# OnurBasci/TransformerBasedNavierStokeSolver

Hardware: AMD Instinct MI355X
Metric: ns64_train_samples_per_s (higher is better)
Workload: dtype f32

## Files before the change

### transformerbasednavierstokesolver_amd/csrc/pa2d_gemm.hip

```cpp
#include "pa2d_gemm_common.h"
#include <string.h>


static Pa2dEnv read_env() {
    auto is = [](const char* n, const char* pre) { const char* e = getenv(n); return e && strncmp(e, pre, strlen(pre)) == 0; };
    auto num = [](const char* n, int dflt) { const char* e = getenv(n); return (e && e[0]) ? atoi(e) : dflt; };
    Pa2dEnv v;
    v.conv_halo = is("PA2D_CONV_HALO", "o") ? 0 : (is("PA2D_CONV_HALO", "f") ? 2 : 1);
    v.mc_big_off = is("PA2D_MC_BIG", "o") ? 1 : 0;
    v.kc_bk16 = num("PA2D_KC_BK", 0) == 16 ? 1 : 0;
    v.mc_bk = num("PA2D_MC_BK", 16) == 32 ? 32 : 16;
    v.mc_splits = num("PA2D_MC_SPLITS", 0);
    v.mcb_splits = num("PA2D_MCB_SPLITS", 0);
    v.lin_dw_split = is("PA2D_LIN_DW_SPLIT", "of") ? 0 : 1;
    v.lin_panel = is("PA2D_LIN_PANEL", "of") ? 0 : 1;
    v.lin_rowpanel = is("PA2D_LIN_ROWPANEL", "of") ? 0 : 1;
    v.lin_small_split = is("PA2D_LIN_SMALL_SPLIT", "of") ? 0 : 1;
    v.conv_mfma16 = num("PA2D_CONV_MFMA", 16) == 32 ? 0 : 1;
    v.conv_ahead = num("PA2D_CONV_AHEAD", 1) == 0 ? 0 : 1;
    v.mc_mfma16 = num("PA2D_MC_MFMA", 16) == 32 ? 0 : 1;
    v.split_big = num("PA2D_SPLIT_BIG", 1);
    v.slice_map = is("PA2D_SLICE_MAP", "l") ? 0 : 1;
    v.default_engine = is("PA2D_GEMM", "f") ? 0 : (is("PA2D_GEMM", "b") ? 2 : 1);
    v.tail_panel = num("PA2D_TAIL_PANEL", 0);
    return v;
}
static Pa2dEnv g_env = read_env();
const Pa2dEnv& pa2d_env() { return g_env; }


static int kc_bk(bool im2col, int Cin) {
    if (im2col && pa2d_env().kc_bk16) return 16;
    return (!im2col || (Cin % 32) == 0) ? 32 : 16;
}
static KCTile kc_tile(int M, int N, bool im2col, int Cin) {
    const int tiles_m = ceil_div(M, 128);
    const long long t128 = (long long)tiles_m * ceil_div(N, 128);
    const long long t12864 = (long long)tiles_m * ceil_div(N, 64);
    const int bk = kc_bk(im2col, Cin);
    if (N > 64 && t128 >= 384) return {128, 128, bk};
    if (t12864 >= 384 || M <= 64) return {128, 64, bk};
    return {64, 64, bk};
}
static bool use_split(int engine, int N, bool im2col, int Cin) {
    const int m = engine;
    if (m == 1) return im2col && N > 64 && (Cin % 32) == 0;
    if (m == 2) return N > 64 && (!im2col || (Cin % 32) == 0);
    return false;
}
static bool kc_split_small_applies(const KCParams& p, bool im2col) {
    if (!pa2d_env().lin_small_split || im2col || p.io_bf16 || p.engine != 1) return false;
    if ((p.K % 32) != 0 || p.K < 64 || p.N < 64 || p.M < 256) return false;
    return (long long)ceil_div(p.M, 128) * ceil_div(p.N, 128) < 384;
}
static int persistent_mode(const KCParams& p) {
    const bool gelu = p.act == ACT_GELU, has_res = p.res != nullptr;
    if (p.epi == 0) return 0;
    if (gelu && !has_res && (p.epi == (EPI_ACT | EPI_STORE_PRE) || p.epi == EPI_ACT)) return 1;
    if (gelu && !has_res && p.epi == EPI_MUL_DACT && !p.bias) return 2;
    return -1;
}
static bool panel_applies(const KCParams& p, bool im2col) {
    if (!pa2d_env().lin_panel || im2col) return false;
    if (p.io_bf16 || (p.engine != 1 && p.engine != 2)) return false;
    if ((p.K % 32) != 0 || p.N < 64) return false;
    if (persistent_mode(p) < 0) return false;
    if (p.epi == EPI_ACT && p.aux) return false;
    return (long long)(p.M / 256) * ceil_div(p.N, 128) >= 256;
}
static size_t rowpanel_image_bytes(int N, int K, int engine) {
    if (engine != 1 || (K != 128 && K != 256) || N < 128 || N > 1024 || (N % 128) != 0) return 0;
    return (size_t)N * K * 6;
}
static bool rowpanel_applies(const KCParams& p) {
    if (!pa2d_env().lin_rowpanel || p.io_bf16) return false;
    if (rowpanel_image_bytes(p.N, p.K, p.engine) == 0) return false;
    if (persistent_mode(p) < 0 || (p.epi == EPI_ACT && p.aux)) return false;
    if ((p.lda & 3) || (p.ldc & 3) || (p.res && (p.ldres & 3)) || (p.aux && (p.ldaux & 3))) return false;
    return p.M / 128 >= 256;
}
static bool conv_halo_applies(const KCParams& p) {
    const int pol = pa2d_env().conv_halo;
    if (p.taps == 27) return false;
    if (pol == 0 || !p.apre || (p.Cin % 32) != 0 || p.H <= 0 || p.W <= 0 || (p.M % (p.H * p.W)) != 0) return false;
    const long long tiles = (long long)(p.M / (p.H * p.W)) * ceil_div(p.H, KC_HALO_TH) * ceil_div(p.W, KC_HALO_TW) * ceil_div(p.N, 128);
    return pol == 2 || tiles >= 512;
}

KCChoice plan_kc(const KCParams& p, bool im2col) {
    KCChoice c = {};
    c.mode = c.tail_family = c.tail_bm = c.tail_bn = -1;
    c.out_bf16 = p.io_bf16;
    c.reads_b = true;
    c.wimg_bytes = im2col ? 0 : rowpanel_image_bytes(p.N, p.K, p.engine);
    const int nt = p.engine == 2 ? 1 : 3;
    if (!im2col && p.wimg && rowpanel_applies(p)) {
        c.family = KC_ROWPANEL; c.bm = 128; c.bn = 64; c.bk = 64; c.nt = 3;
    } else if (panel_applies(p, im2col)) {
        c.family = KC_PANEL; c.bm = 256; c.bn = 128; c.bk = 32; c.nt = nt;
    } else if (p.io_bf16 || use_split(p.engine, p.N, im2col, p.Cin)) {
        c.family = KC_SPLIT; c.bm = 128; c.bn = 128; c.bk = 32; c.nt = nt;
        c.a_planes = im2col ? p.apre != 0 : p.io_bf16 != 0;
        if (im2col) c.pack = KC_PACK_PLANES;
        if (im2col ? !p.apre : p.engine != 2) c.rc = PA2D_ERR_ARG;
        else if (p.io_bf16 && (p.taps == 27 || p.engine != 2 || (!im2col && (p.K % 32) != 0))) c.rc = PA2D_ERR_UNSUPPORTED;
        else if (im2col && conv_halo_applies(p)) {
            c.family = KC_HALO; c.bm = 256;
            c.mfma16 = nt == 3 && pa2d_env().conv_mfma16 && (p.N % 4) == 0 && (p.ldc % 4) == 0;
            c.ahead = c.mfma16 && pa2d_env().conv_ahead;
        } else if (im2col && !p.io_bf16 && nt == 3) {
            const int tiles_n = ceil_div(p.N, 128);
            if (pa2d_env().split_big && (p.M % 256) == 0 && (long long)(p.M / 256) * tiles_n >= 512) c.bm = 256;
            else if ((long long)ceil_div(p.M, 128) * tiles_n < 256) c.bm = 64;
        }
    } else if (kc_split_small_applies(p, im2col)) {
        c.family = KC_SPLIT_SMALL; c.bm = 64; c.bn = 64; c.bk = 32; c.nt = 3;
    } else {
        const KCTile t = kc_tile(p.M, p.N, im2col, p.Cin);
        c.family = KC_EXACT; c.bm = t.bm; c.bn = t.bn; c.bk = t.bk;
        if (im2col) c.pack = t.bk == 32 ? KC_PACK_F32_32 : KC_PACK_F32_16;
    }
    if (c.family == KC_PANEL || c.family == KC_ROWPANEL) {
        c.mode = persistent_mode(p);
        c.head_rows = p.M - p.M % c.bm;
        if (c.head_rows < p.M) {
            KCParams pt = p;
            pt.wimg = nullptr;
            pt.M = p.M - c.head_rows;
            const KCChoice t = plan_kc(pt, false);
            c.tail_family = t.family; c.tail_bm = t.bm; c.tail_bn = t.bn;
        }
        c.reads_b = c.family == KC_PANEL || c.head_rows < p.M;
    }
    return c;
}

static bool kc_extents(KCParams& p, bool im2col, const KCChoice& c) {
    const unsigned long long lim = 0xFFFFFFF0ull;
    const unsigned long long es = p.io_bf16 ? 2ull : 4ull;
    unsigned long long ab = ((unsigned long long)(p.M - 1) * p.lda + (im2col ? p.Cin : p.K)) * 4ull;
    unsigned long long bb = ((unsigned long long)(p.N - 1) * p.ldb + p.K) * 4ull;
    const unsigned long long cb = ((unsigned long long)(p.M - 1) * p.ldc + p.N) * es;
    const unsigned long long rb = p.res ? ((unsigned long long)(p.M - 1) * p.ldres + p.N) * es : 0ull;
    const unsigned long long xb = p.aux ? ((unsigned long long)(p.M - 1) * p.ldaux + p.N) * es : 0ull;
    if (ab >= lim || bb >= lim || cb >= lim || rb >= lim || xb >= lim) return false;
    if (c.a_planes) ab = im2col ? (unsigned long long)p.M * (p.Cin / 32) * c.nt * 64 : ab / 2;
    if (c.pack == KC_PACK_PLANES) bb = (unsigned long long)p.N * (p.K / 32) * c.nt * 64;
    if (ab >= lim) return false;
    p.a_bytes = (unsigned)ab; p.b_bytes = (unsigned)bb;
    p.c_bytes = (unsigned)cb; p.res_bytes = (unsigned)rb; p.aux_bytes = (unsigned)xb;
    return true;
}

static int launch_head_tail(const KCParams& p_in, const KCParams& p, const KCChoice& c, hipStream_t st) {
    int rc;
    if (c.family == KC_ROWPANEL && p.wsrc) {
        rc = launch_pack_weight_image(p.wsrc, p.wsn, p.wsk, p.wimg, p.N, p.K, st);
        if (rc) return rc;
    }
    KCParams ph = p;
    ph.M = c.head_rows;
    rc = c.family == KC_ROWPANEL ? launch_kc_rowpanel(ph, c, st) : launch_kc_panel(ph, c, st);
    if (rc || c.head_rows == p.M) return rc;
    KCParams pt = p_in;
    pt.wimg = nullptr;
    pt.M = p.M - c.head_rows;
    pt.A = p.A + (size_t)c.head_rows * p.lda;
    pt.C = p.C + (size_t)c.head_rows * p.ldc;
    if (p.res) pt.res = p.res + (size_t)c.head_rows * p.ldres;
    if (p.aux) pt.aux = p.aux + (size_t)c.head_rows * p.ldaux;
    return launch_kc(pt, false, st);
}

// ... 258 lines not shown
```

### transformerbasednavierstokesolver_amd/csrc/pa2d_gemm_mc_planes.hip

```cpp
#include "pa2d_gemm_common.h"
#include "pa2d_bf16_split.h"

struct MCPlanesParams {
    const void* PA; int chA;
    const void* PB; int chB;
    float* slab;
    int Mi, Nj, Mk, chunks_per_split, splits, H, W, Cin;
    unsigned a_bytes, b_bytes;
    int taps;
    long long lda, ldb;
    float* colsum;
};

__device__ __forceinline__ unsigned img_off(int row, int ch) {
    return 256u * row + 16u * (ch ^ (((row & 3) << 2) | ((row >> 2) & 3)));
}

#define MC16_FRAG(base_, t_, pl_)                                                                         \
    __builtin_bit_cast(bf16x8, __builtin_shufflevector(                                                   \
        __builtin_amdgcn_ds_read_tr16_b64_v4i16((lds_s16x4*)(smem + ((base_[0] ^ ((unsigned)(t_) << 5)) + (pl_) * PIMG))), \
        __builtin_amdgcn_ds_read_tr16_b64_v4i16((lds_s16x4*)(smem + ((base_[1] ^ ((unsigned)(t_) << 5)) + (pl_) * PIMG))), \
        0, 1, 2, 3, 4, 5, 6, 7))

template <int NT, int KS, bool F32SRC = false, bool MF16 = false>
// ... 108 lines not shown
    _Pragma("unroll") for (int op = 0; op < 2; ++op) MC_SPLIT_ROW8(NT, rg[op * 2], rg[op * 2 + 1], op == 0 && do_cs, cs, pk[op])
#define MP16_WRITE(buf_)                                                                                  \
    _Pragma("unroll") for (int op = 0; op < 2; ++op) _Pragma("unroll") for (int pl = 0; pl < NT; ++pl)    \
        *reinterpret_cast<bf16x8*>(smem + (buf_) * STAGE + flds + (op * NT + pl) * PIMG) = pk[op][pl];
        const int nst = c_end - c_begin, steps = (nst + 1) >> 1;
        if (nst > 0) {
            MP_LOAD(c_begin)
            MP16_CONVERT()
            MP16_WRITE(0)
            MP_LOAD(c_begin + 1)
            MP16_CONVERT()
            MP16_WRITE(1)
            if (steps > 1) { MP_LOAD(c_begin + 2) }
        }
        __syncthreads();
        int sp = 0, sq = 1, sr = 2;
        for (int k = 0; k < steps; ++k) {
            const bool has_next = k + 1 < steps;
            const unsigned lo = (unsigned)((kq >> 1) ? sq : sp) * (unsigned)STAGE;
            const unsigned ua[2] = {fa[0] + lo, fa[1] + lo};
            const unsigned ub[2] = {fb[0] + lo + NT * PIMG, fb[1] + lo + NT * PIMG};
            bf16x8 xf[4][NT];
#pragma unroll
            for (int j = 0; j < 4; ++j)
#pragma unroll
                for (int pl = 0; pl < NT; ++pl) xf[j][pl] = MC16_FRAG(ub, j, pl);
            bf16x8 afc[NT], afn[NT];
#pragma unroll
            for (int pl = 0; pl < NT; ++pl) afc[pl] = MC16_FRAG(ua, 0, pl);
#pragma unroll
            for (int ib = 0; ib < 4; ++ib) {
                if (ib < 3) {
#pragma unroll
                    for (int pl = 0; pl < NT; ++pl) afn[pl] = MC16_FRAG(ua, ib + 1, pl);
                }
                if (ib == 1 && has_next) {
                    MP16_CONVERT()
                    MP16_WRITE(sr)
                    MP_LOAD(c_begin + 2 * k + 3)
                }
                if (ib == 3) {
                    if (has_next) {
                        MP16_CONVERT()
                        if (k + 2 < steps) { MP_LOAD(c_begin + 2 * k + 4) }
                    }
                    __syncthreads();
                    if (has_next) { MP16_WRITE(sp) }
                }
                MP16_MMA(ib, afc)
#pragma unroll
                for (int pl = 0; pl < NT; ++pl) afc[pl] = afn[pl];
            }
            __syncthreads();
            const int t = sp;
            sp = sr;
            sr = sq;
            sq = t;
        }
#undef MP16_CONVERT
#undef MP16_WRITE
#undef MP16_MMA
        if (do_cs) {
            float* sm = reinterpret_cast<float*>(smem);
#pragma unroll
            for (int e = 0; e < 8; ++e) sm[frow * 128 + fc8 * 8 + e] = cs[e];
            mc_colsum_reduce<128, 16>(sm, tid, ti, split, p.Mi, p.colsum);
        }
        float* out = p.slab + (size_t)split * p.Mi * p.Nj;
#pragma unroll
        for (int j = 0; j < 4; ++j) {
            const int col = tj * 128 + wn * 64 + j * 16 + 4 * kq;
#pragma unroll
            for (int ib = 0; ib < 4; ++ib) {
                const int row = ti * 128 + wm * 64 + ib * 16 + (lane & 15);
                if (row < p.Mi && col < p.Nj) *reinterpret_cast<f32x4*>(out + (size_t)row * p.Nj + col) = acc[ib][j];
            }
        }
        return;
    }

    f32x16 acc[2][2];
#pragma unroll
    for (int i = 0; i < 2; ++i)
#pragma unroll
        for (int j = 0; j < 2; ++j)
#pragma unroll
            for (int r = 0; r < 16; ++r) acc[i][j][r] = 0.f;

    const int g = lane >> 4, q4 = (lane & 15) >> 2, pq = lane & 3;
    unsigned fa[2][2], fb[2][2];
#pragma unroll
    for (int t = 0; t < 2; ++t)
#pragma unroll
        for (int r = 0; r < 2; ++r) {
            const int row = 8 * (g >> 1) + 4 * r + q4;
            const int cha = ((wm * 64 + t * 32) >> 3) + 2 * (g & 1) + (pq >> 1);
            const int chb = ((wn * 64 + t * 32) >> 3) + 2 * (g & 1) + (pq >> 1);
            fa[t][r] = img_off(row, cha) + 8u * (pq & 1);
            fb[t][r] = img_off(row, chb) + 8u * (pq & 1);
        }

    if (c_begin < c_end) {
        MP_LOAD(c_begin)
        MP_STORE(0)
    }
    __syncthreads();
    for (int c = c_begin; c < c_end; c += KS) {
        const int buf = ((c - c_begin) / KS) & 1;
        if (c + KS < c_end) { MP_LOAD(c + KS) }
#pragma unroll
        for (int ks = 0; ks < KS; ++ks) {
        const unsigned char* st = smem + buf * STAGE + ks * PIMG;
        bf16x8 af[2][NT], bf[2][NT];
#pragma unroll
        for (int t = 0; t < 2; ++t)
#pragma unroll
            for (int pl = 0; pl < NT; ++pl) {
                af[t][pl] = tr_frag(st + pl * KS * PIMG, fa[t][0], fa[t][1]);
                bf[t][pl] = tr_frag(st + (NT + pl) * KS * PIMG, fb[t][0], fb[t][1]);
            }
#pragma unroll
        for (int i = 0; i < 2; ++i)
#pragma unroll
            for (int j = 0; j < 2; ++j) split_terms(af[i], bf[j], acc[i][j]);
        }
        if (c + KS < c_end) { MP_STORE(buf ^ 1) }
        __syncthreads();
    }
#undef MP_LOAD
#undef MP_STORE

    if constexpr (F32SRC) {
        if (do_cs) {
            float* sm = reinterpret_cast<float*>(smem);
#pragma unroll
            for (int e = 0; e < 8; ++e) sm[frow * 128 + fc8 * 8 + e] = cs[e];
            mc_colsum_reduce<128, 16>(sm, tid, ti, split, p.Mi, p.colsum);
        }
    }
    float* out = p.slab + (size_t)split * p.Mi * p.Nj;
    const int col0 = tj * 128 + wn * 64 + (lane & 31);
    const int row0 = ti * 128 + wm * 64 + 4 * (lane >> 5);
#pragma unroll
    for (int j = 0; j < 2; ++j)
#pragma unroll
        for (int i = 0; i < 2; ++i)
#pragma unroll
            for (int r = 0; r < 16; ++r) {
                const int row = row0 + i * 32 + (r & 3) + 8 * (r >> 2);
                if (!F32SRC || (row < p.Mi && col0 + j * 32 < p.Nj)) out[(size_t)row * p.Nj + col0 + j * 32] = acc[i][j][r];
            }
}

template <int NT, int KS, bool MF16 = false>
__global__ __launch_bounds__(512, 1) void gemm_mc_planes_big_kernel(const MCPlanesParams p, const int per_xcd) {
    constexpr int PIMG = 8192;
    constexpr int STAGE = 2 * NT * KS * PIMG;
    constexpr int NP = (2 * NT * KS * 512) / 512;
    extern __shared__ __attribute__((aligned(16))) unsigned char smem[];

    const int tid = threadIdx.x, lane = tid & 63, wave = tid >> 6;
    const int tiles_i = (p.Mi + 255) / 256, tiles_j = (p.Nj + 255) / 256;
    const int tiles = tiles_i * tiles_j;
    const int lin = (blockIdx.x & 7) * per_xcd + (blockIdx.x >> 3);
    if ((int)(blockIdx.x >> 3) >= per_xcd || lin >= tiles * p.splits) return;
    const int split = lin / tiles, t_ = lin - split * tiles;
    const int ti = t_ / tiles_j, tj = t_ - ti * tiles_j;
    const int wm = wave >> 2, wn = wave & 3;
    const int total_chunks = (p.Mk + 15) / 16;
    const int c_begin = split * p.chunks_per_split;
    const int c_end = min(total_chunks, c_begin + p.chunks_per_split);
    const int HW = p.taps == 1 ? 1 : p.H * p.W;

    const __amdgpu_buffer_rsrc_t ra_rsrc = __builtin_amdgcn_make_buffer_rsrc(const_cast<void*>(p.PA), 0, p.a_bytes, 0x00020000);
    const __amdgpu_buffer_rsrc_t rb_rsrc = __builtin_amdgcn_make_buffer_rsrc(const_cast<void*>(p.PB), 0, p.b_bytes, 0x00020000);

    const int row16 = tid >> 5, cgrp = (tid & 31) >> 2, piece = tid & 3;
    const bool colok_a = ti * 256 + cgrp * 32 < p.Mi;
    const unsigned goff_a = (unsigned)((((ti * 256) >> 5) + cgrp) * NT * 64 + piece * 16);
    const int jc = tj * 256 + cgrp * 32;
    const int tap = p.taps == 1 ? 4 : jc / p.Cin;
    const bool colok_b = jc < p.Nj;
    const unsigned goff_b = (unsigned)((p.taps == 1 ? (jc >> 5) : ((jc - tap * p.Cin) >> 5)) * NT * 64 + piece * 16);
    const int tap_dy = tap / 3 - 1, tap_dx = tap - (tap / 3) * 3 - 1, tap_shift = tap_dy * p.W + tap_dx;
    const unsigned pitch_a = (unsigned)(p.chA * NT * 64), pitch_b = (unsigned)(p.chB * NT * 64);
    const unsigned lds_off = 512u * row16 + 16u * ((unsigned)(cgrp * 4 + piece) ^ (unsigned)(((row16 & 3) << 2) | ((row16 >> 2) & 3)));
#define MB_LOAD(c_, RG)                                                                                   \
    {                                                                                                     \
        _Pragma("unroll") for (int ks = 0; ks < KS; ++ks) {                                               \
            const int m_ = ((c_) + ks) * 16 + row16;                                                      \
            const bool okr_ = m_ < p.Mk && (c_) + ks < c_end;             \
            bool okb_ = okr_ && colok_b;                                                                  \
            int mm_ = m_;                                                                                 \
            if (p.taps != 1) {       \
                okb_ = okb_ && (unsigned)(ly + tap_dy) < (unsigned)p.H && (unsigned)(lx + tap_dx) < (unsigned)p.W; \
                mm_ = m_ + tap_shift;                                                                     \
                lx += 16;                                                                                 \
                while (lx >= p.W) { lx -= p.W; ++ly; }                                                    \
                while (ly >= p.H) ly -= p.H;                                                              \
            }                                                                                             \
            const unsigned oa_ = (okr_ && colok_a) ? (unsigned)m_ * pitch_a + goff_a : OOB_OFF;           \
            const unsigned ob_ = okb_ ? (unsigned)mm_ * pitch_b + goff_b : OOB_OFF;                       \
            _Pragma("unroll") for (int pl = 0; pl < NT; ++pl) {                                           \
                RG[pl * KS + ks] = __builtin_amdgcn_raw_buffer_load_b128(ra_rsrc, oa_ == OOB_OFF ? OOB_OFF : oa_ + pl * 64u, 0, 0); \
                RG[(NT + pl) * KS + ks] = __builtin_amdgcn_raw_buffer_load_b128(rb_rsrc, ob_ == OOB_OFF ? OOB_OFF : ob_ + pl * 64u, 0, 0); \
            }                                                                                             \
        }                                                                                                 \
    }
#define MB_STORE(buf_, RG)                                                                                \
    {                                                                                                     \
        _Pragma("unroll") for (int s = 0; s < NP; ++s)                                                    \
            *reinterpret_cast<u32x4*>(smem + (buf_) * STAGE + s * PIMG + lds_off) = RG[s];                \
    }
    u32x4 rg0[NP];
    int ly = 0, lx = 0;
    if (p.taps != 1) {
        const int n0 = (c_begin * 16 + row16) % HW;
        ly = n0 / p.W;
        lx = n0 - ly * p.W;
    }

    if constexpr (MF16) {
        static_assert(NT == 3 && KS == 1, "the 16x16x32 form is written for the split engine");
        f32x4 acc[8][4];
#pragma unroll
        for (int i = 0; i < 8; ++i)
#pragma unroll
            for (int j = 0; j < 4; ++j) acc[i][j] = f32x4{0.f, 0.f, 0.f, 0.f};
        const int kq = lane >> 4, q4 = (lane & 15) >> 2, pq = lane & 3;
        unsigned fa[2], fb[2];
#pragma unroll
        for (int r = 0; r < 2; ++r) {
            const int row = 8 * (kq & 1) + 4 * r + q4;
            const unsigned swz = (unsigned)(((row & 3) << 2) | ((row >> 2) & 3));
            fa[r] = 512u * row + 16u * ((unsigned)(wm * 16 + (pq >> 1)) ^ swz) + 8u * (pq & 1);
            fb[r] = 512u * row + 16u * ((unsigned)(wn * 8 + (pq >> 1)) ^ swz) + 8u * (pq & 1);
        }
#define MB16_MMA(ib_, AF) _Pragma("unroll") for (int j = 0; j < 4; ++j) split_terms(AF, xf[j], acc[ib_][j]);
        const int nst = c_end - c_begin, steps = (nst + 1) >> 1;
        if (nst > 0) {
            MB_LOAD(c_begin, rg0)
            MB_STORE(0, rg0)
            MB_LOAD(c_begin + 1, rg0)
            MB_STORE(1, rg0)
            if (steps > 1) MB_LOAD(c_begin + 2, rg0)
        }
        __syncthreads();
        int sp = 0, sq = 1, sr = 2;
        for (int k = 0; k < steps; ++k) {
            const unsigned lo = (unsigned)((kq >> 1) ? sq : sp) * (unsigned)STAGE;
            const unsigned ua[2] = {fa[0] + lo, fa[1] + lo};
            const unsigned ub[2] = {fb[0] + lo + NT * PIMG, fb[1] + lo + NT * PIMG};
            bf16x8 xf[4][NT];
#pragma unroll
            for (int j = 0; j < 4; ++j)
#pragma unroll
                for (int pl = 0; pl < NT; ++pl) xf[j][pl] = MC16_FRAG(ub, j, pl);
            bf16x8 afc[NT], afn[NT];
#pragma unroll
            for (int pl = 0; pl < NT; ++pl) afc[pl] = MC16_FRAG(ua, 0, pl);
#pragma unroll
            for (int ib = 0; ib < 8; ++ib) {
                if (ib < 7) {
#pragma unroll
                    for (int pl = 0; pl < NT; ++pl) afn[pl] = MC16_FRAG(ua, ib + 1, pl);
                }
                if (ib == 4) {
                    MB_STORE(sr, rg0)
                    MB_LOAD(c_begin + 2 * k + 3, rg0)
                }
                if (ib == 7) {
                    __syncthreads();
                    MB_STORE(sp, rg0)
                    MB_LOAD(c_begin + 2 * k + 4, rg0)
                }
                MB16_MMA(ib, afc)
#pragma unroll
                for (int pl = 0; pl < NT; ++pl) afc[pl] = afn[pl];
            }
            __syncthreads();
            const int t = sp;
            sp = sr;
            sr = sq;
            sq = t;
        }
#undef MB16_MMA
        float* out = p.slab + (size_t)split * p.Mi * p.Nj;
#pragma unroll
        for (int j = 0; j < 4; ++j) {
            const int col = tj * 256 + wn * 64 + j * 16 + 4 * kq;
            if (col >= p.Nj) continue;
#pragma unroll
            for (int ib = 0; ib < 8; ++ib) {
                const int row = ti * 256 + wm * 128 + ib * 16 + (lane & 15);
                if (row < p.Mi) *reinterpret_cast<f32x4*>(out + (size_t)row * p.Nj + col) = acc[ib][j];
            }
        }
        return;
    }

    f32x16 acc[4][2];
#pragma unroll
    for (int i = 0; i < 4; ++i)
#pragma unroll
        for (int j = 0; j < 2; ++j)
#pragma unroll
            for (int r = 0; r < 16; ++r) acc[i][j][r] = 0.f;

    const int g = lane >> 4, q4 = (lane & 15) >> 2, pq = lane & 3;
    unsigned fa[4][2], fb[2][2];
#pragma unroll
    for (int r = 0; r < 2; ++r) {
        const int row = 8 * (g >> 1) + 4 * r + q4;
        const unsigned swz = (unsigned)(((row & 3) << 2) | ((row >> 2) & 3));
#pragma unroll
        for (int t = 0; t < 4; ++t) {
            const int cha = ((wm * 128 + t * 32) >> 3) + 2 * (g & 1) + (pq >> 1);
            fa[t][r] = 512u * row + 16u * ((unsigned)cha ^ swz) + 8u * (pq & 1);
        }
#pragma unroll
        for (int t = 0; t < 2; ++t) {
            const int chb = ((wn * 64 + t * 32) >> 3) + 2 * (g & 1) + (pq >> 1);
            fb[t][r] = 512u * row + 16u * ((unsigned)chb ^ swz) + 8u * (pq & 1);
        }
    }

#define MB_COMPUTE(buf_)                                                                                  \
    _Pragma("unroll") for (int ks = 0; ks < KS; ++ks) {                                                   \
        const unsigned char* st = smem + (buf_) * STAGE + ks * PIMG;                                      \
        bf16x8 af[4][NT], bf[2][NT];                                                                      \
        _Pragma("unroll") for (int pl = 0; pl < NT; ++pl) {                                               \
            _Pragma("unroll") for (int t = 0; t < 4; ++t)                                                 \
                af[t][pl] = tr_frag(st + pl * KS * PIMG, fa[t][0], fa[t][1]);                             \
            _Pragma("unroll") for (int t = 0; t < 2; ++t)                                                 \
                bf[t][pl] = tr_frag(st + (NT + pl) * KS * PIMG, fb[t][0], fb[t][1]);                      \
        }                                                                                                 \
        _Pragma("unroll") for (int i = 0; i < 4; ++i)                                                     \
            _Pragma("unroll") for (int j = 0; j < 2; ++j) split_terms(af[i], bf[j], acc[i][j]);           \
    }
    if (c_begin < c_end) {
        MB_LOAD(c_begin, rg0)
        MB_STORE(0, rg0)
        if (c_begin + KS < c_end) MB_LOAD(c_begin + KS, rg0)
    }
    __syncthreads();
    for (int c = c_begin; c < c_end; c += KS) {
        const int buf = ((c - c_begin) / KS) & 1;
        if (c + KS < c_end) {
            MB_STORE(buf ^ 1, rg0)
            if (c + 2 * KS < c_end) MB_LOAD(c + 2 * KS, rg0)
        }
        MB_COMPUTE(buf)
        __syncthreads();
    }
#undef MB_COMPUTE
#undef MB_LOAD
#undef MB_STORE

    float* out = p.slab + (size_t)split * p.Mi * p.Nj;
    const int col0 = tj * 256 + wn * 64 + (lane & 31);
    const int row0 = ti * 256 + wm * 128 + 4 * (lane >> 5);
    MC_STORE_TILES(4, 2)
}

template <typename K>
static int launch_big(K kernel, int smem, const MCPlanesParams& p, int wgs, hipStream_t st) {
    const int per_xcd = ceil_div(wgs, 8);
    return launch_lds(kernel, dim3(per_xcd * 8), dim3(512), smem, st, p, per_xcd);
}

int launch_wgrad_planes(const MCDesc& d, const MCChoice& c, unsigned a_bytes, unsigned b_bytes, float* slab, hipStream_t st) {
    const int NT = d.engine == 2 ? 1 : 3;
    const bool mf16 = NT == 3 && pa2d_env().mc_mfma16 && (reinterpret_cast<uintptr_t>(slab) & 15) == 0;
    MCPlanesParams p = {};
    p.PA = d.A; p.PB = d.B; p.slab = slab; p.a_bytes = a_bytes; p.b_bytes = b_bytes;
    p.Mi = d.Mi; p.Nj = d.Nj; p.Mk = d.Mk; p.chunks_per_split = c.pl.chunks_per_split; p.splits = c.pl.splits;
    p.H = d.H; p.W = d.W; p.Cin = d.Cin; p.taps = d.taps;
    if (c.kernel == MC_K_PLANES256) {
        p.chA = d.Mi / 32; p.chB = d.Cin / 32;
        const int wgs = ceil_div(p.Mi, 256) * ceil_div(p.Nj, 256) * c.pl.splits;
        int rc;
        if (mf16) rc = launch_big(&gemm_mc_planes_big_kernel<3, 1, true>, 3 * 2 * 3 * 1 * 8192, p, wgs, st);
        else if (NT == 3) rc = launch_big(&gemm_mc_planes_big_kernel<3, 1>, 2 * 2 * 3 * 1 * 8192, p, wgs, st);
        else rc = launch_big(&gemm_mc_planes_big_kernel<1, 4>, 2 * 2 * 1 * 4 * 8192, p, wgs, st);
        return rc;
    }
    if (!c.pl.big) return PA2D_ERR_UNSUPPORTED;
    const dim3 grid(ceil_div(d.Mi, 128) * ceil_div(d.Nj, 128) * c.pl.splits);
    if (c.kernel == MC_K_PLANES128) {
        if ((d.Mi % 128) || (d.Cin % 128) || d.taps != 9) return PA2D_ERR_UNSUPPORTED;
        p.chA = d.Mi / 32; p.chB = d.Cin / 32;
        if (NT == 3) hipLaunchKernelGGL((gemm_mc_planes_kernel<3, 1>), grid, dim3(256), 0, st, p);
        else hipLaunchKernelGGL((gemm_mc_planes_kernel<1, 4>), grid, dim3(256), 0, st, p);
    } else {
        p.lda = d.lda; p.ldb = d.ldb; p.colsum = d.colsum;
        if (mf16 && (d.Nj % 4) == 0) hipLaunchKernelGGL((gemm_mc_planes_kernel<3, 1, true, true>), grid, dim3(256), 0, st, p);
        else if (NT == 3) hipLaunchKernelGGL((gemm_mc_planes_kernel<3, 1, true>), grid, dim3(256), 0, st, p);
        else hipLaunchKernelGGL((gemm_mc_planes_kernel<1, 4, true>), grid, dim3(256), 0, st, p);
    }
    PA2D_CHECK_LAUNCH();
    return PA2D_OK;
}
```

### transformerbasednavierstokesolver_amd/csrc/pa2d_internal.h

```cpp
#pragma once
#include <hip/hip_runtime.h>
#include <stdint.h>

typedef float f32x16 __attribute__((ext_vector_type(16)));
typedef float f32x4 __attribute__((ext_vector_type(4)));

#define PA2D_OK 0
#define PA2D_ERR_ARG 1001
#define PA2D_ERR_UNSUPPORTED 1002
#define PA2D_ERR_WORKSPACE 1003

#define PA2D_CHECK_LAUNCH()                         \
    do {                                            \
        hipError_t e__ = hipGetLastError();         \
        if (e__ != hipSuccess) return (int)e__;     \
    } while (0)

enum { ACT_NONE = 0, ACT_GELU = 1, ACT_TANH = 2, ACT_SIGMOID = 3, ACT_RELU = 4, ACT_SOFTPLUS = 5,
       ACT_ELU = 6, ACT_SILU = 7 };

__device__ __forceinline__ float normal_cdf(float x, float& e_out) {
#pragma clang fp contract(off)
    const float z = fabsf(x) * 0.70710678118654752440f;
    const float t = __builtin_amdgcn_rcpf(fmaf(0.3275911f, z, 1.0f));
    float poly = fmaf(1.061405429f, t, -1.453152027f);
    poly = fmaf(poly, t, 1.421413741f);
    poly = fmaf(poly, t, -0.284496736f);
    poly = fmaf(poly, t, 0.254829592f);
    const float e = __builtin_amdgcn_exp2f(-z * z * 1.44269504088896340736f);
    e_out = e;
    const float hq = 0.5f * poly * t * e;
    return x < 0.f ? hq : 1.0f - hq;
}
__device__ __forceinline__ float gelu_exact(float x) {
#pragma clang fp contract(off)
    float e;
    return x * normal_cdf(x, e);
}
__device__ __forceinline__ float dgelu_exact(float x) {
#pragma clang fp contract(off)
    float e;
    const float cdf = normal_cdf(x, e);
    return fmaf(x * 0.39894228040143267794f, e, cdf);
}

__device__ __forceinline__ float act_fwd(int id, float x) {
    switch (id) {
        case ACT_GELU: return gelu_exact(x);
        case ACT_TANH: return tanhf(x);
        case ACT_SIGMOID: return 1.0f / (1.0f + expf(-x));
        case ACT_RELU: return x > 0.f ? x : 0.f;
        case ACT_SOFTPLUS: return x > 20.f ? x : log1pf(expf(x));
        case ACT_ELU: return x > 0.f ? x : expm1f(x);
        case ACT_SILU: return x / (1.0f + expf(-x));
        default: return x;
    }
}

__device__ __forceinline__ float act_bwd(int id, float x) {
    switch (id) {
        case ACT_GELU: return dgelu_exact(x);
        case ACT_TANH: { const float t = tanhf(x); return 1.0f - t * t; }
        case ACT_SIGMOID: { const float s = 1.0f / (1.0f + expf(-x)); return s * (1.0f - s); }
        case ACT_RELU: return x > 0.f ? 1.f : 0.f;
        case ACT_SOFTPLUS: return x > 20.f ? 1.f : 1.0f / (1.0f + expf(-x));
        case ACT_ELU: return x > 0.f ? 1.f : expf(x);
        case ACT_SILU: { const float s = 1.0f / (1.0f + expf(-x)); return s * (1.0f + x * (1.0f - s)); }
        default: return 1.f;
    }
}

__device__ __forceinline__ float wave_sum(float v) {
#pragma unroll
    for (int o = 32; o > 0; o >>= 1) v += __shfl_xor(v, o, 64);
    return v;
}
__device__ __forceinline__ float wave_max(float v) {
#pragma unroll
    for (int o = 32; o > 0; o >>= 1) v = fmaxf(v, __shfl_xor(v, o, 64));
    return v;
}

typedef unsigned int u32x4 __attribute__((ext_vector_type(4)));
#define OOB_OFF 0xFFFFFFFFu

__device__ __forceinline__ __amdgpu_buffer_rsrc_t make_rsrc(const float* base, unsigned bytes) {
    return __builtin_amdgcn_make_buffer_rsrc(const_cast<float*>(base), 0, bytes, 0x00020000);
}
__device__ __forceinline__ float4 buf_load4(__amdgpu_buffer_rsrc_t r, unsigned voff) {
    const u32x4 v = __builtin_amdgcn_raw_buffer_load_b128(r, voff, 0, 0);
    return make_float4(__uint_as_float(v.x), __uint_as_float(v.y), __uint_as_float(v.z), __uint_as_float(v.w));
}


__device__ __forceinline__ float buf_load1(__amdgpu_buffer_rsrc_t r, unsigned voff) {
    return __uint_as_float(__builtin_amdgcn_raw_buffer_load_b32(r, voff, 0, 0));
}
__device__ __forceinline__ void buf_store1(__amdgpu_buffer_rsrc_t r, unsigned voff, float v) {
    __builtin_amdgcn_raw_buffer_store_b32(__float_as_uint(v), r, voff, 0, 0);
}

__device__ __forceinline__ float2 buf_load2(__amdgpu_buffer_rsrc_t r, unsigned voff) {
    typedef unsigned int u32x2_ __attribute__((ext_vector_type(2)));
    const u32x2_ v = __builtin_amdgcn_raw_buffer_load_b64(r, voff, 0, 0);
    return make_float2(__uint_as_float(v.x), __uint_as_float(v.y));
}
__device__ __forceinline__ void buf_store4(__amdgpu_buffer_rsrc_t r, unsigned voff, float4 v) {
    u32x4 u = {__float_as_uint(v.x), __float_as_uint(v.y), __float_as_uint(v.z), __float_as_uint(v.w)};
    __builtin_amdgcn_raw_buffer_store_b128(u, r, voff, 0, 0);
}

#define PA2D_ACT_SAVE_DERIVATIVE_BIT 0x100

struct Pa2dEnv {
    int conv_halo;
    int mc_big_off;
    int kc_bk16;
    int mc_bk;
    int mc_splits;
    int mcb_splits;
    int lin_dw_split;
    int lin_panel;
    int conv_mfma16;
    int conv_ahead;
    int mc_mfma16;
    int lin_small_split;
    int lin_rowpanel;
    int split_big;
    int slice_map;
    int default_engine;
    int tail_panel;
};
const Pa2dEnv& pa2d_env();

static inline int pa2d_zero(void* p, size_t bytes, hipStream_t st) {
    if (!p || !bytes) return PA2D_OK;
    return (int)hipMemsetAsync(p, 0, bytes, st);
}
static inline int ceil_div(int a, int b) { return (a + b - 1) / b; }
static inline long long ceil_div_ll(long long a, long long b) { return (a + b - 1) / b; }

struct ReduceSegs { int nseg; long long begin[5]; float* dst[4]; };
int pa2d_launch_reduce_segs(const float* slab, int nslab, long long count, const ReduceSegs& segs, int accumulate,
                            hipStream_t st);

typedef __bf16 bf16_t;
template <typename T> struct Act;
template <> struct Act<float> {
    static constexpr unsigned ES = 4;
    static __device__ __forceinline__ float4 ld4(const float* p) { return *reinterpret_cast<const float4*>(p); }
    static __device__ __forceinline__ void st4(float* p, float4 v) { *reinterpret_cast<float4*>(p) = v; }
    static __device__ __forceinline__ float ld1(const float* p) { return *p; }
    static __device__ __forceinline__ float4 bld4(__amdgpu_buffer_rsrc_t r, unsigned off) { return buf_load4(r, off); }
    static __device__ __forceinline__ float2 bld2(__amdgpu_buffer_rsrc_t r, unsigned off) { return buf_load2(r, off); }
    static __device__ __forceinline__ float bld1(__amdgpu_buffer_rsrc_t r, unsigned off) { return buf_load1(r, off); }
    static __device__ __forceinline__ float bld1s(__amdgpu_buffer_rsrc_t r, unsigned off, unsigned soff) {
        return __uint_as_float(__builtin_amdgcn_raw_buffer_load_b32(r, off, soff, 0));
    }
    static __device__ __forceinline__ void bst4(__amdgpu_buffer_rsrc_t r, unsigned off, float4 v) { buf_store4(r, off, v); }
    static __device__ __forceinline__ void bst1(__amdgpu_buffer_rsrc_t r, unsigned off, float v) { buf_store1(r, off, v); }
};
__device__ __forceinline__ float bf16_bits_to_f32(unsigned short b) { return __uint_as_float((unsigned)b << 16); }
__device__ __forceinline__ unsigned short f32_to_bf16_bits(float x) {
    const bf16_t h = (bf16_t)x;
    return __builtin_bit_cast(unsigned short, h);
}
__device__ __forceinline__ unsigned pack_bf16x2(float lo, float hi) {
    return (unsigned)f32_to_bf16_bits(lo) | ((unsigned)f32_to_bf16_bits(hi) << 16);
}
template <> struct Act<bf16_t> {
    static constexpr unsigned ES = 2;
    static __device__ __forceinline__ float4 unpack4(uint2 q) {
        return make_float4(__uint_as_float(q.x << 16), __uint_as_float(q.x & 0xFFFF0000u), __uint_as_float(q.y << 16),
                           __uint_as_float(q.y & 0xFFFF0000u));
    }
    static __device__ __forceinline__ float4 ld4(const bf16_t* p) { return unpack4(*reinterpret_cast<const uint2*>(p)); }
    static __device__ __forceinline__ void st4(bf16_t* p, float4 v) {
        *reinterpret_cast<uint2*>(p) = make_uint2(pack_bf16x2(v.x, v.y), pack_bf16x2(v.z, v.w));
    }
    static __device__ __forceinline__ float ld1(const bf16_t* p) { return (float)*p; }
    static __device__ __forceinline__ float4 bld4(__amdgpu_buffer_rsrc_t r, unsigned off) {
        typedef unsigned int u32x2_ __attribute__((ext_vector_type(2)));
        const u32x2_ q = __builtin_amdgcn_raw_buffer_load_b64(r, off, 0, 0);
        return unpack4(make_uint2(q.x, q.y));
    }
    static __device__ __forceinline__ float2 bld2(__amdgpu_buffer_rsrc_t r, unsigned off) {
        const unsigned q = __builtin_amdgcn_raw_buffer_load_b32(r, off, 0, 0);
        return make_float2(__uint_as_float(q << 16), __uint_as_float(q & 0xFFFF0000u));
    }
    static __device__ __forceinline__ float bld1(__amdgpu_buffer_rsrc_t r, unsigned off) {
        return bf16_bits_to_f32(__builtin_amdgcn_raw_buffer_load_b16(r, off, 0, 0));
    }
    static __device__ __forceinline__ float bld1s(__amdgpu_buffer_rsrc_t r, unsigned off, unsigned soff) {
        return bf16_bits_to_f32(__builtin_amdgcn_raw_buffer_load_b16(r, off, soff, 0));
    }
    static __device__ __forceinline__ void bst4(__amdgpu_buffer_rsrc_t r, unsigned off, float4 v) {
        typedef unsigned int u32x2_ __attribute__((ext_vector_type(2)));
        const u32x2_ q = {pack_bf16x2(v.x, v.y), pack_bf16x2(v.z, v.w)};
        __builtin_amdgcn_raw_buffer_store_b64(q, r, off, 0, 0);
    }
    static __device__ __forceinline__ void bst1(__amdgpu_buffer_rsrc_t r, unsigned off, float v) {
        __builtin_amdgcn_raw_buffer_store_b16(f32_to_bf16_bits(v), r, off, 0, 0);
    }
};
__device__ __forceinline__ __amdgpu_buffer_rsrc_t make_rsrc_v(const void* base, unsigned bytes) {
    return __builtin_amdgcn_make_buffer_rsrc(const_cast<void*>(base), 0, bytes, 0x00020000);
}

__device__ __forceinline__ bool slice_decode(int xcd_map, int B, int heads, int nchunk, int& b, int& hh, int& chunk, int& bid) {
    const int total = B * heads * nchunk;
    int L;
    if (xcd_map) {
        const int per = (total + 7) >> 3;
        if ((int)(blockIdx.x >> 3) >= per) return false;
        L = (int)(blockIdx.x & 7) * per + (int)(blockIdx.x >> 3);
        if (L >= total) return false;
        hh = L % heads;
        chunk = (L / heads) % nchunk;
        b = L / (heads * nchunk);
    } else {
        L = (int)blockIdx.x;
        if (L >= total) return false;
        chunk = L % nchunk;
        hh = (L / nchunk) % heads;
        b = L / (nchunk * heads);
    }
    bid = (b * heads + hh) * nchunk + chunk;
    return true;
}
static inline int slice_grid(int total) { return ((total + 7) / 8) * 8; }
```

Baseline: 71.62.

## Stage big multi-channel GEMM tiles via buffer-load-to-LDS DMA with chained MFMA issue

Adds a DMA staging path for the 256x256 multi-channel planes GEMM kernel. Global tiles are loaded straight into LDS with buffer_load ... lds (inline asm driving m0) rather than through registers and ds_write. The XOR swizzle moves into the per-thread source chunk index, and A fragments are preloaded into a larger register array. An optional chained mode puts scheduling barriers between MFMA groups. Both are on by default via env flags; this frees VGPRs and removes LDS store instructions, at the cost of hand-written asm, a changed sync placement and more register use for A fragments.

```diff
diff --git a/transformerbasednavierstokesolver_amd/csrc/pa2d_gemm.hip b/transformerbasednavierstokesolver_amd/csrc/pa2d_gemm.hip
--- a/transformerbasednavierstokesolver_amd/csrc/pa2d_gemm.hip
+++ b/transformerbasednavierstokesolver_amd/csrc/pa2d_gemm.hip
@@ -19,6 +19,8 @@
     v.conv_mfma16 = num("PA2D_CONV_MFMA", 16) == 32 ? 0 : 1;
     v.conv_ahead = num("PA2D_CONV_AHEAD", 1) == 0 ? 0 : 1;
     v.mc_mfma16 = num("PA2D_MC_MFMA", 16) == 32 ? 0 : 1;
+    v.mc_dma = num("PA2D_MC_DMA", 1) == 0 ? 0 : 1;
+    v.mc_chain = num("PA2D_MC_CHAIN", 1) == 0 ? 0 : 1;
     v.split_big = num("PA2D_SPLIT_BIG", 1);
     v.slice_map = is("PA2D_SLICE_MAP", "l") ? 0 : 1;
     v.default_engine = is("PA2D_GEMM", "f") ? 0 : (is("PA2D_GEMM", "b") ? 2 : 1);
diff --git a/transformerbasednavierstokesolver_amd/csrc/pa2d_gemm_mc_planes.hip b/transformerbasednavierstokesolver_amd/csrc/pa2d_gemm_mc_planes.hip
--- a/transformerbasednavierstokesolver_amd/csrc/pa2d_gemm_mc_planes.hip
+++ b/transformerbasednavierstokesolver_amd/csrc/pa2d_gemm_mc_planes.hip
@@ -284,7 +284,10 @@
             }
 }
 
-template <int NT, int KS, bool MF16 = false>
+#ifndef MB_MID
+#define MB_MID 5
+#endif
+template <int NT, int KS, bool MF16 = false, bool DMA = false, bool CHAIN = false>
 __global__ __launch_bounds__(512, 1) void gemm_mc_planes_big_kernel(const MCPlanesParams p, const int per_xcd) {
     constexpr int PIMG = 8192;
     constexpr int STAGE = 2 * NT * KS * PIMG;
@@ -307,7 +310,11 @@
     const __amdgpu_buffer_rsrc_t ra_rsrc = __builtin_amdgcn_make_buffer_rsrc(const_cast<void*>(p.PA), 0, p.a_bytes, 0x00020000);
     const __amdgpu_buffer_rsrc_t rb_rsrc = __builtin_amdgcn_make_buffer_rsrc(const_cast<void*>(p.PB), 0, p.b_bytes, 0x00020000);
 
-    const int row16 = tid >> 5, cgrp = (tid & 31) >> 2, piece = tid & 3;
+    static_assert(!DMA || MF16, "LDS-DMA staging is written for the 16x16x32 pipeline");
+    static_assert(!CHAIN || DMA, "the chained issue order needs the registers that DMA staging frees");
+    const int row16 = tid >> 5;
+    const int lchunk = DMA ? (tid & 31) ^ (((row16 & 3) << 2) | ((row16 >> 2) & 3)) : (tid & 31);
+    const int cgrp = lchunk >> 2, piece = lchunk & 3;
     const bool colok_a = ti * 256 + cgrp * 32 < p.Mi;
     const unsigned goff_a = (unsigned)((((ti * 256) >> 5) + cgrp) * NT * 64 + piece * 16);
     const int jc = tj * 256 + cgrp * 32;
@@ -344,7 +351,45 @@
         _Pragma("unroll") for (int s = 0; s < NP; ++s)                                                    \
             *reinterpret_cast<u32x4*>(smem + (buf_) * STAGE + s * PIMG + lds_off) = RG[s];                \
     }
-    u32x4 rg0[NP];
+#define MB_DMA(c_, buf_)                                                                                  \
+    {                                                                                                     \
+        const int m_ = (c_) * 16 + row16;                                                                 \
+        const bool okr_ = m_ < p.Mk && (c_) < c_end;                                                      \
+        bool okb_ = okr_ && colok_b;                                                                      \
+        int mm_ = m_;                                                                                     \
+        if (p.taps != 1) {                                                                                \
+            okb_ = okb_ && (unsigned)(ly + tap_dy) < (unsigned)p.H && (unsigned)(lx + tap_dx) < (unsigned)p.W; \
+            mm_ = m_ + tap_shift;                                                                         \
+            lx += 16;                                                                                     \
+            while (lx >= p.W) { lx -= p.W; ++ly; }                                                        \
+            while (ly >= p.H) ly -= p.H;                                                                  \
+        }                                                                                                 \
+        const unsigned oa_ = (okr_ && colok_a) ? (unsigned)m_ * pitch_a + goff_a : OOB_OFF;               \
+        const unsigned ob_ = okb_ ? (unsigned)mm_ * pitch_b + goff_b : OOB_OFF;                           \
+        const unsigned va_[NT] = {oa_, oa_ == OOB_OFF ? OOB_OFF : oa_ + 64u, oa_ == OOB_OFF ? OOB_OFF : oa_ + 128u}; \
+        const unsigned vb_[NT] = {ob_, ob_ == OOB_OFF ? OOB_OFF : ob_ + 64u, ob_ == OOB_OFF ? OOB_OFF : ob_ + 128u}; \
+        unsigned keep_;                                                                                   \
+        asm volatile(MB_DMA_ASM                                                                           \
+                     : "=&s"(keep_)                                                                       \
+                     : "s"(lds_base + (unsigned)(buf_) * (unsigned)STAGE), "s"(dma_ra), "s"(dma_rb),      \
+                       "v"(va_[0]), "v"(va_[1]), "v"(va_[2]), "v"(vb_[0]), "v"(vb_[1]), "v"(vb_[2])       \
+                     : "memory", "scc");                                                                  \
+    }
+#define MB_DMA_ASM                                                                                        \
+    "s_nop 4\n\ts_mov_b32 %0, m0\n\ts_mov_b32 m0, %1\n\ts_nop 0\n\t"                                      \
+    "buffer_load_dwordx4 %4, %2, 0 offen lds\n\ts_add_u32 m0, m0, 0x2000\n\ts_nop 0\n\t"                  \
+    "buffer_load_dwordx4 %5, %2, 0 offen lds\n\ts_add_u32 m0, m0, 0x2000\n\ts_nop 0\n\t"                  \
+    "buffer_load_dwordx4 %6, %2, 0 offen lds\n\ts_add_u32 m0, m0, 0x2000\n\ts_nop 0\n\t"                  \
+    "buffer_load_dwordx4 %7, %3, 0 offen lds\n\ts_add_u32 m0, m0, 0x2000\n\ts_nop 0\n\t"                  \
+    "buffer_load_dwordx4 %8, %3, 0 offen lds\n\ts_add_u32 m0, m0, 0x2000\n\ts_nop 0\n\t"                  \
+    "buffer_load_dwordx4 %9, %3, 0 offen lds\n\ts_mov_b32 m0, %0"
+#define MB_DMA_WAIT() asm volatile("s_waitcnt vmcnt(0)" ::: "memory")
+    static_assert(!DMA || (NT == 3 && PIMG == 0x2000), "MB_DMA_ASM is written out for six 8 KB images");
+    typedef __attribute__((address_space(3))) unsigned char lds_char;
+    const unsigned lds_base = (unsigned)(uintptr_t)(lds_char*)smem + (unsigned)__builtin_amdgcn_readfirstlane(wave) * 1024u;
+    const u32x4 dma_ra = {(unsigned)(uintptr_t)p.PA, (unsigned)((uintptr_t)p.PA >> 32) & 0xFFFFu, p.a_bytes, 0x00020000u};
+    const u32x4 dma_rb = {(unsigned)(uintptr_t)p.PB, (unsigned)((uintptr_t)p.PB >> 32) & 0xFFFFu, p.b_bytes, 0x00020000u};
+    u32x4 rg0[DMA ? 1 : NP];
     int ly = 0, lx = 0;
     if (p.taps != 1) {
         const int n0 = (c_begin * 16 + row16) % HW;
@@ -368,14 +413,25 @@
             fa[r] = 512u * row + 16u * ((unsigned)(wm * 16 + (pq >> 1)) ^ swz) + 8u * (pq & 1);
             fb[r] = 512u * row + 16u * ((unsigned)(wn * 8 + (pq >> 1)) ^ swz) + 8u * (pq & 1);
         }
-#define MB16_MMA(ib_, AF) _Pragma("unroll") for (int j = 0; j < 4; ++j) split_terms(AF, xf[j], acc[ib_][j]);
+#define MB16_MMA(ib_, AF)                                                                                 \
+    _Pragma("unroll") for (int j = 0; j < 4; ++j) {                                                       \
+        split_terms(AF, xf[j], acc[ib_][j]);                                                              \
+        if constexpr (CHAIN) MB16_CHAIN_PIN(j)                                                            \
+    }
+#define MB16_CHAIN_PIN(j_) __builtin_amdgcn_sched_barrier(0);
         const int nst = c_end - c_begin, steps = (nst + 1) >> 1;
         if (nst > 0) {
-            MB_LOAD(c_begin, rg0)
-            MB_STORE(0, rg0)
-            MB_LOAD(c_begin + 1, rg0)
-            MB_STORE(1, rg0)
-            if (steps > 1) MB_LOAD(c_begin + 2, rg0)
+            if constexpr (DMA) {
+                MB_DMA(c_begin, 0)
+                MB_DMA(c_begin + 1, 1)
+                MB_DMA_WAIT();
+            } else {
+                MB_LOAD(c_begin, rg0)
+                MB_STORE(0, rg0)
+                MB_LOAD(c_begin + 1, rg0)
+                MB_STORE(1, rg0)
+                if (steps > 1) MB_LOAD(c_begin + 2, rg0)
+            }
         }
         __syncthreads();
         int sp = 0, sq = 1, sr = 2;
@@ -388,6 +444,27 @@
             for (int j = 0; j < 4; ++j)
 #pragma unroll
                 for (int pl = 0; pl < NT; ++pl) xf[j][pl] = MC16_FRAG(ub, j, pl);
+            if constexpr (DMA) {
+                bf16x8 af[8][NT];
+#pragma unroll
+                for (int pl = 0; pl < NT; ++pl) af[0][pl] = MC16_FRAG(ua, 0, pl);
+#pragma unroll
+                for (int ib = 0; ib < 8; ++ib) {
+#pragma unroll
+                    for (int t = 1; t < 8; ++t)
+                        if (ib + 1 == (t < MB_MID ? t : MB_MID)) {
+#pragma unroll
+                            for (int pl = 0; pl < NT; ++pl) af[t][pl] = MC16_FRAG(ua, t, pl);
+                        }
+                    if (ib == 1) MB_DMA(c_begin + 2 * k + 2, sr)
+                    if (ib == MB_MID) {
+                        __syncthreads();
+                        MB_DMA(c_begin + 2 * k + 3, sp)
+                    }
+                    MB16_MMA(ib, af[ib])
+                }
+                MB_DMA_WAIT();
+            } else {
             bf16x8 afc[NT], afn[NT];
 #pragma unroll
             for (int pl = 0; pl < NT; ++pl) afc[pl] = MC16_FRAG(ua, 0, pl);
@@ -410,6 +487,7 @@
 #pragma unroll
                 for (int pl = 0; pl < NT; ++pl) afc[pl] = afn[pl];
             }
+            }
             __syncthreads();
             const int t = sp;
             sp = sr;
@@ -417,6 +495,7 @@
             sq = t;
         }
 #undef MB16_MMA
+#undef MB16_CHAIN_PIN
         float* out = p.slab + (size_t)split * p.Mi * p.Nj;
 #pragma unroll
         for (int j = 0; j < 4; ++j) {
@@ -488,6 +567,9 @@
 #undef MB_COMPUTE
 #undef MB_LOAD
 #undef MB_STORE
+#undef MB_DMA
+#undef MB_DMA_ASM
+#undef MB_DMA_WAIT
 
     float* out = p.slab + (size_t)split * p.Mi * p.Nj;
     const int col0 = tj * 256 + wn * 64 + (lane & 31);
@@ -512,7 +594,10 @@
         p.chA = d.Mi / 32; p.chB = d.Cin / 32;
         const int wgs = ceil_div(p.Mi, 256) * ceil_div(p.Nj, 256) * c.pl.splits;
         int rc;
-        if (mf16) rc = launch_big(&gemm_mc_planes_big_kernel<3, 1, true>, 3 * 2 * 3 * 1 * 8192, p, wgs, st);
+        const int dma = mf16 ? (pa2d_env().mc_dma ? (pa2d_env().mc_chain ? 2 : 1) : 0) : 0;
+        if (dma == 2) rc = launch_big(&gemm_mc_planes_big_kernel<3, 1, true, true, true>, 3 * 2 * 3 * 1 * 8192, p, wgs, st);
+        else if (dma == 1) rc = launch_big(&gemm_mc_planes_big_kernel<3, 1, true, true>, 3 * 2 * 3 * 1 * 8192, p, wgs, st);
+        else if (mf16) rc = launch_big(&gemm_mc_planes_big_kernel<3, 1, true>, 3 * 2 * 3 * 1 * 8192, p, wgs, st);
         else if (NT == 3) rc = launch_big(&gemm_mc_planes_big_kernel<3, 1>, 2 * 2 * 3 * 1 * 8192, p, wgs, st);
         else rc = launch_big(&gemm_mc_planes_big_kernel<1, 4>, 2 * 2 * 1 * 4 * 8192, p, wgs, st);
         return rc;
diff --git a/transformerbasednavierstokesolver_amd/csrc/pa2d_internal.h b/transformerbasednavierstokesolver_amd/csrc/pa2d_internal.h
--- a/transformerbasednavierstokesolver_amd/csrc/pa2d_internal.h
+++ b/transformerbasednavierstokesolver_amd/csrc/pa2d_internal.h
@@ -124,6 +124,8 @@
     int conv_mfma16;
     int conv_ahead;
     int mc_mfma16;
+    int mc_dma;
+    int mc_chain;
     int lin_small_split;
     int lin_rowpanel;
     int split_big;
```

Result: faster. 73.04, median of 6 (+2.0%).
